# pminervini/hyperopt

Hardware: AMD Instinct MI355X
Metric: EI candidates scored/sec (x components) (higher is better)
Workload: dtype f64 (log-sum-exp: fp64 accumulation, fp32 exp2 of the shifted term, its argument from an fp32 block-local quadratic (mode 3); quantized: fp64 erf); 1 GPU; config 4: 100-D uniform space, 1e4-trial history, 1e7 candidates/suggest (lpdf roofline stress); parallelism=single

## Files before the change

### hyperopt_amd/csrc/tpe_engine.hip

```cpp
#include <hip/hip_runtime.h>

#include <algorithm>
#include <cmath>
#include <cstdlib>
#include <cstdio>
#include <cstring>
#include <string>
#include <vector>

#include "tpe_anneal.hpp"
#include "tpe_group_plan.hpp"
#include "tpe_internal.hpp"
#include "tpe_level_plan.hpp"
#include "tpe_pareto_plan.hpp"
#include "tpe_hv_plan.hpp"
#include "tpe_switches.hpp"

using namespace tpe;
static_assert(sizeof(AnnealTrace) == sizeof(tpe_anneal_trace), "layout");

struct tpe_engine {
  int32_t device = 0;
  hipStream_t stream = nullptr;
  static constexpr int kAux = 4;
// ... 697 lines not shown
  return TPE_OK;
}

StepShape step_shape(const tpe_plan *p, int64_t n_sug, int64_t n_cand, int64_t cand_begin,
                     int64_t n_total, int32_t last_nb, const FitVariant &f) {
  StepShape s;
  s.n_sug = n_sug;
  s.n_cand = n_cand;
  s.cand_begin = cand_begin;
  s.n_total = n_total;
  s.below = below_class(last_nb >= 0 ? (int64_t)last_nb + 1 : p->kcap);
  s.fit = f;
  s.prune_mode = p->prune_mode;
  s.lattice_on = p->lattice_on;
  s.screen_run = step_screen_run(switches());
  s.table_lean = switches().table_lean;
  return s;
}

int run_level(tpe_engine *h, tpe_plan *p, int level, const StepShape &s, hipStream_t st) {
  const LevelPlan lp = plan_level(*p, switches(), s, level);
  const int64_t n_sug = s.n_sug;
  const int32_t n_level = lp.n_level, n_lat = lp.n_lat;
  const int32_t *lvl = p->d_level_hps + p->level_off[level];
  if (lp.empty) {
    if (n_level > 0) CKH(launch_merge(lvl, n_level, (int32_t)n_sug, p->P, 0, nullptr, p->d_results, st));
    return TPE_OK;
  }
  ScoreArgs la = base_args(p, n_sug);
  la.level_hps = lvl;
// ... 117 lines not shown
      case Draw::Plain:
        CKH(launch_draw(a, c.table_draw, st));
        break;
      default: {
        hipError_t e;
        if (c.draw == Draw::Sorted) {
          e = launch_draw_sorted(a, c.small_table, c.fast, p->d_cpos, st);
        } else {
          rc = table_build(h, p, st);
          if (rc) { join_lk(); return rc; }
          p->tab_pstride = a.pstride;
          e = launch_draw_sorted(a, c.small_table, c.fast, p->d_cpos, st, 1);
          if (e == hipSuccess) e = launch_table_pilot(a, st);
          if (c.draw == Draw::SortedScreened) {
            if (e == hipSuccess)
              e = launch_draw_zone(a, p->d_draw_zone, c.screen_tiles, kScreenMargin, c.screen_guide,
                                   st);
            if (e == hipSuccess)
              e = launch_draw_screened(a, p->d_cpos, p->d_draw_zone, p->d_screen_stats,
                                       c.screen_guide >= 0, c.screen_run, st);
          } else if (e == hipSuccess) {
            e = launch_draw_pruned(a, c.small_table, c.fast, p->d_cpos, st);
          }
        }
        if (e != hipSuccess) { join_lk(); return fail(h, TPE_E_HIP, hipGetErrorString(e)); }
        p->dump_cn = cn;
        p->dump_sstride = a.cand_sstride;
        p->dump_level = level;
        p->dump_nsug = n_sug;
      }
    }
    a.tab_pref = c.tab_pref;
    if (c.bucket) CKH(launch_bucket(a, n_lat, p->d_cpos, st));
    a.cand_pos = c.cand_pos ? p->d_cpos : nullptr;
    if (!joined) {
// ... 2659 lines not shown
```

### hyperopt_amd/csrc/tpe_internal.hpp

```cpp
#pragma once
#include <hip/hip_runtime.h>
#include <stdint.h>

#include "../../include/tpe_engine.h"

namespace tpe {

constexpr double kEPS = 1e-12;
constexpr int kFitThreads = 1024;
constexpr int kScoreThreads = 256;
constexpr int kMaxLeaves = 160;

enum { KIND_LSE_G = 0, KIND_LSE_L = 1, KIND_ERF_G = 2, KIND_ERF_L = 3, KIND_CAT = 4,
       KIND_LAT = 5, KIND_LSE_G1 = 6, KIND_LSE_L1 = 7, KIND_LSE_GW = 8, KIND_LSE_LW = 9,
       KIND_LSE_GW1 = 10, KIND_LSE_LW1 = 11 };
constexpr int64_t kWaveRowSplitMax = (int64_t)1 << 18;

__host__ __device__ constexpr bool kind_lse(int k) {
  return k == KIND_LSE_G || k == KIND_LSE_L || k == KIND_LSE_G1 || k == KIND_LSE_L1 ||
         k == KIND_LSE_GW || k == KIND_LSE_LW || k == KIND_LSE_GW1 || k == KIND_LSE_LW1;
}
__host__ __device__ constexpr bool kind_logn(int k) {
  return k == KIND_LSE_L || k == KIND_LSE_L1 || k == KIND_LSE_LW || k == KIND_LSE_LW1 ||
         k == KIND_ERF_L;
// ... 309 lines not shown
constexpr int kZoneEdges = 2 * kZoneMax - 2;
constexpr double kScreenMargin = 1.6e-5;
constexpr int kGuideBitsMax = 10;
struct __attribute__((aligned(16))) DrawZone {
  int32_t nz;
  int32_t gbits;
  double gap_lo[kZoneMax - 1];
  double gap_hi[kZoneMax - 1];
  double thr[kFuseTab][kZoneEdges];
  uint64_t thrI[kFuseTab][kZoneEdges];
  uint64_t pickB[kFuseTab];
  uint16_t guide[1 << kGuideBitsMax];
  double tcdf[kFuseTab], tbase[kFuseTab], tmass[kFuseTab];
  unsigned char tmode[kFuseTab];
};
hipError_t launch_draw_zone(const ScoreArgs &a, DrawZone *zones, int32_t tiles, double margin,
                            int32_t guide_bits, hipStream_t st);
constexpr int kScreenRunMax = 16;
hipError_t launch_draw_screened(const ScoreArgs &a, int32_t *pos_out, const DrawZone *zones,
                                unsigned long long *stats, bool integer, int32_t run,
                                hipStream_t st);
bool is_screen_draw_kernel_fn(const void *f);
bool is_screen_run_kernel_fn(const void *f);
hipError_t launch_table_pilot(const ScoreArgs &a, hipStream_t st);
static_assert(kSortedBlock == TPE_SHARD_ALIGN, "shard alignment is the sorted-draw block");
hipError_t launch_sort_ext(const ScoreArgs &a, const double *src, int32_t *pos_out,
                           hipStream_t st);
hipError_t launch_bucket(const ScoreArgs &a, int32_t slot_begin, int32_t *pos_out, hipStream_t st);
hipError_t launch_publish(const void *src, void *dst, size_t bytes, uint64_t *flag, uint64_t seq,
                          hipStream_t st);
hipError_t launch_merge(const int32_t *level_hps, int32_t n_slots,
                        int32_t n_suggest, int32_t n_hp, int32_t world,
                        const Partial *gathered, Partial *results,
                        hipStream_t st, Partial *out2 = nullptr);
hipError_t launch_sample(const tpe_hp *hp_dev, const double *mw,
// ... 335 lines not shown
```

### hyperopt_amd/csrc/tpe_level_plan.hpp

```cpp
#pragma once
#include <algorithm>
#include <cstdint>
#include <utility>
#include <vector>

#include "tpe_internal.hpp"
#include "tpe_switches.hpp"

namespace tpe {

constexpr int64_t kSortedDrawMin = (int64_t)1 << 22;
constexpr int64_t kSmallSortMin = 2048;
constexpr int64_t kTileDrawMax = 4096;

inline int32_t active_bound(const std::vector<tpe_hp> &all, const std::vector<int32_t> &cond_parent,
                            const std::vector<int32_t> &cond_branch, const int32_t *hps, int b,
                            int e) {
  int32_t n = 0;
  std::vector<std::pair<int32_t, int32_t>> pb;
  for (int i = b; i < e; ++i) {
    const tpe_hp &x = all[hps[i]];
    if (x.cond_count == 0) { ++n; continue; }
    std::vector<std::pair<int32_t, int32_t>> mine;
    for (int c = 0; c < x.cond_count; ++c)
// ... 115 lines not shown
  f.mom_w = moments ? mom_width(ps, sw, n_hist) : 0;
  f.mom_h = f.mom_w == 16;
  return f;
}

struct StepShape {
  int64_t n_sug = 0, n_cand = 0, cand_begin = 0;
  int64_t n_total = 0;
  int32_t below = BELOW_LARGE;
  FitVariant fit;
  int32_t prune_mode = 3;
  bool lattice_on = true;
  bool capturing = false;
  bool publish = false;
  int32_t screen_run = 0;
  bool table_lean = true;
  bool operator==(const StepShape &o) const {
    return n_sug == o.n_sug && n_cand == o.n_cand && cand_begin == o.cand_begin &&
           n_total == o.n_total && below == o.below && fit == o.fit &&
           prune_mode == o.prune_mode && lattice_on == o.lattice_on &&
           capturing == o.capturing && publish == o.publish && screen_run == o.screen_run &&
           table_lean == o.table_lean;
  }
};
inline int32_t step_screen_run(const Switches &sw) {
  return sw.draw_screen && sw.draw_screen_int ? (int32_t)sw.draw_screen_run : 0;
}

struct ScoreGrid {
  int32_t n_groups = 0, pstride = 1;
  int32_t grp_kind[kMaxGroups] = {}, grp_slot0[kMaxGroups] = {}, grp_tiles[kMaxGroups] = {};
  int32_t grp_block0[kMaxGroups + 1] = {}, grp_slots[kMaxGroups] = {};
  int32_t blocks() const { return grp_block0[n_groups]; }
};
template <typename Kind, typename Rows>
ScoreGrid score_grid(Kind kind, int n_slots, int64_t cn, Rows rows) {
  ScoreGrid g;
  int32_t blocks = 0;
  auto weight = [](int k) {
    if (k == KIND_ERF_G || k == KIND_ERF_L) return 0;
    if (kind_lse(k)) return 1;
// ... 47 lines not shown
  SortedPruned,
  SortedScreened,
};

struct ChunkPlan {
  int64_t c0 = 0, cn = 0;
  bool accumulate = false;
  ScoreGrid grid;
  int32_t sort_log2 = 0, lse_pos = 0, lse_prune = 0, lse_f32 = 0, lookup_draw = 0;
  bool lk_fork = false;
  Draw draw = Draw::Plain;
  bool table_draw = false;
  bool small_table = false;
  bool fast = false;
  int32_t screen_tiles = 0;
  int32_t screen_guide = -1;
  int32_t screen_run = 0;
  bool bucket = false;
  bool cand_pos = false;
  int32_t tab_on = 0, tab_pref = 0;
  int classes = 7;
  bool publish = false;
};

struct LevelPlan {
  bool empty = false;
  int32_t n_level = 0;
  int32_t n_lat = 0;
  int32_t lat_rows = 0;
  bool compact = false;
// ... 102 lines not shown
      c.draw = Draw::Fused;
    } else if (sorted) {
      c.fast = true;
      for (int i = 0; i < n_level && c.fast; ++i) {
        const tpe_hp &x = ps.hps[hl[i]];
        const bool lookup = i < n_lat || L.kinds[i] == KIND_CAT;
        c.fast = lookup ? c.lookup_draw != 0
                        : (x.family != TPE_CAT && (x.flags & TPE_HAS_LOW) && (x.flags & TPE_HAS_HIGH));
      }
      const bool prune = c.tab_on == 1 && c.tab_pref && (cls & 1) && sw.draw_prune &&
                         c.sort_log2 == kSortLog2Large && c.cn > kSortedBlock;
      const bool screen = prune && c.fast && small_table && sw.draw_screen &&
                          c.cn * n_sug * n_level >= sw.draw_screen_min;
      c.draw = screen ? Draw::SortedScreened : prune ? Draw::SortedPruned : Draw::Sorted;
      c.screen_tiles = (int32_t)sw.draw_screen_tiles;
      c.screen_guide = sw.draw_screen_int ? (int32_t)sw.draw_screen_guide_bits : -1;
      c.screen_run = screen && c.screen_guide >= 0 ? s.screen_run : 0;
      if (prune) c.tab_pref = 2;
    } else {
      c.draw = Draw::Plain;
    }
    c.bucket = (lp.erf_level || small_sort) && !sorted;
    c.cand_pos = lp.erf_level || sorted || small_sort;
    lp.chunks.push_back(c);
  }
  return lp;
}

}
```

### hyperopt_amd/csrc/tpe_screen.hip

```cpp
#include <float.h>
#include <math.h>

#include "tpe_draw.hpp"
#include "tpe_internal.hpp"
#include "tpe_philox_row.hpp"

namespace tpe {

constexpr double kScreenQMin = 0x1p-24;
constexpr int kScreenThreads = 512;
constexpr int kZoneThreads = 256;
constexpr int kZoneCand = kHotIv + 2;
constexpr int kScreenList = 640;

__device__ __forceinline__ bool zone_crossed(double u1, double b, double m, int md, double z,
                                             double tail, bool up) {
  double pu, pp, q1;
  {
#pragma clang fp contract(off)
    const double um = u1 * m;
    pu = b - um;
    pp = b + um;
    q1 = 1.0 - pp;
  }
// ... 4 lines not shown
    above = pu < t_lo;
    below = pu > t_hi;
  } else if (md == 2 || z < 0.0) {
    above = pp > t_hi;
    below = pp < t_lo;
  } else {
    above = pp >= 0.5 && q1 < t_lo;
    below = pp < 0.5 || q1 > t_hi;
  }
  const bool ok_lo = md == 1 || pp >= kScreenQMin;
  const bool deep_hi = md == 1 ? pu < kScreenQMin : md == 0 && pp >= 0.5 && q1 < kScreenQMin;
  return deep_hi || (ok_lo && (up ? above : !below));
}

__global__ __launch_bounds__(kZoneThreads) void k_draw_zone(ScoreArgs A, DrawZone *zones,
                                                            int32_t tiles, double margin,
                                                            int32_t gbits) {
  __shared__ DrawTableT<kFuseTab> T;
  __shared__ double tmin[kPilotWaves], tmax[kPilotWaves];
  __shared__ double zlo[kZoneCand], zhi[kZoneCand];
  __shared__ uint64_t pb[kFuseTab];
  __shared__ int nz_s, bad_s;
  const int s = blockIdx.y;
  const int slot = row_slot(A, s, 0, A.n_slots, blockIdx.x);
  if (slot < 0) return;
  const int hp = A.level_hps[slot];
  const tpe_hp H = A.hps[hp];
  if (!A.force_active && !A.compact &&
      !hp_active(H, A.results + (int64_t)s * A.n_hp, A.cond_parent, A.cond_branch))
    return;
  const int kind = slot_kind(A, slot);
  if ((kind == KIND_CAT || kind == KIND_LAT) && lookup_inline(A, A.info[2 * hp].K)) return;
  DrawZone *Z = zones + ((int64_t)s * A.n_hp + hp);
  const int t = threadIdx.x, lane = t & 63, wv = t >> 6;
// ... 10 lines not shown
  }
  if (!scr) {
    if (t == 0) Z->nz = 0;
    return;
  }
  const double *pc = A.cand + (int64_t)s * A.cand_sstride + (int64_t)slot * A.n_cand;
  for (int w = wv; w < kPilotWaves; w += kZoneThreads / 64) {
    const double a = pc[w * 128 + lane], b = pc[w * 128 + 64 + lane];
    double mn = fmin(a, b), mx = fmax(a, b);
#pragma unroll
    for (int o = 32; o > 0; o >>= 1) {
      mn = fmin(mn, __shfl_xor(mn, o, 64));
      mx = fmax(mx, __shfl_xor(mx, o, 64));
    }
    if (lane == 0) { tmin[w] = mn; tmax[w] = mx; }
  }
  __syncthreads();
  if (t == 0) {
    const double pm = H.prior_mu, y_lo = hot->y_lo, y_hi = hot->y_hi;
    int nz = 0;
    zlo[nz] = -INFINITY; zhi[nz] = tmax[0]; ++nz;
    zlo[nz] = tmin[kPilotWaves - 1]; zhi[nz] = INFINITY; ++nz;
    for (int j = 0; j < nh; ++j) {
      const double l = hot->lo[j], h = hot->hi[j];
      const double a = l <= y_lo ? -INFINITY : (l + pm) - 8.0 * DBL_EPSILON * (fabs(l) + fabs(pm));
      const double b = h >= y_hi ? INFINITY : (h + pm) + 8.0 * DBL_EPSILON * (fabs(h) + fabs(pm));
      int tf = 0, tl = kPilotWaves - 1;
      while (tf < kPilotWaves && !(tmax[tf] >= a)) ++tf;
      while (tl >= 0 && !(tmin[tl] <= b)) --tl;
      double za = a, zb = b;
      if (a != -INFINITY) {
        const int w = tf - tiles;
        za = w < 0 ? -INFINITY : w < kPilotWaves ? fmin(a, tmin[w]) : a;
      }
      if (b != INFINITY) {
        const int w = tl + tiles;
        zb = w >= kPilotWaves ? INFINITY : w >= 0 ? fmax(b, tmax[w]) : b;
      }
      zlo[nz] = za; zhi[nz] = zb; ++nz;
    }
    for (int i = 1; i < nz; ++i)
      for (int j = i; j > 0 && zlo[j] < zlo[j - 1]; --j) {
        const double a = zlo[j], b = zhi[j];
        zlo[j] = zlo[j - 1]; zhi[j] = zhi[j - 1];
        zlo[j - 1] = a; zhi[j - 1] = b;
      }
    int m = 0;
    for (int i = 1; i < nz; ++i) {
      if (zlo[i] <= zhi[m]) zhi[m] = fmax(zhi[m], zhi[i]);
      else { ++m; zlo[m] = zlo[i]; zhi[m] = zhi[i]; }
    }
    nz = m + 1;
// ... 103 lines not shown
    double run = 0.0;
    for (int e = 0; e < E; ++e) {
      run = fmax(run, Z->thr[k][e]);
      Z->thr[k][e] = run;
    }
    if (gbits >= 0) {
      uint64_t runI = 0;
      for (int e = 0; e < E; ++e) {
        runI = max(runI, Z->thrI[k][e]);
        Z->thrI[k][e] = runI;
      }
    }
  }
}

hipError_t launch_draw_zone(const ScoreArgs &a, DrawZone *zones, int32_t tiles, double margin,
                            int32_t guide_bits, hipStream_t st) {
  const int64_t sbk = (int64_t)1 << a.sort_log2;
  if (a.n_slots <= 0 || a.n_suggest <= 0 || a.n_cand <= sbk) return hipSuccess;
  if (sbk != kSortedBlock || sbk != kPilotWaves * 128 || !zones || !a.tab_hot || !a.tab_hdr ||
      tiles < 0 || guide_bits > kGuideBitsMax)
    return hipErrorInvalidValue;
  k_draw_zone<<<dim3((unsigned)a.slot_rows, a.n_suggest), kZoneThreads, 0, st>>>(
      a, zones, tiles, margin, guide_bits < 0 ? -1 : guide_bits);
  return hipGetLastError();
}

template <int NT>
struct ScreenLds {
  DrawTableT<kFuseTab> T;
  union {
    double thr[kFuseTab * kZoneEdges];
    uint64_t thrI[kFuseTab * kZoneEdges];
  };
  uint32_t cnt[NT / 64 * kSortBuckets / 2];
  double red[2][NT / 64];
  unsigned char hotb[kSortBuckets], liveb[kSortBuckets];
  unsigned long long keep;
  int fail;
  int gapc[NT / 64][kZoneMax - 1];
  int ncl[NT / 64];
  double cx[NT / 64][kScreenList];
  uint32_t ci[NT / 64][kScreenList];
  uint64_t pickB[kFuseTab];
  uint16_t guide[1 << kGuideBitsMax];
};
template <int CAP, int NT>
union ScreenUnion {
  PruneDrawLds<CAP, NT> P;
  ScreenLds<NT> S;
};
static_assert(sizeof(ScreenUnion<kFuseTab, kScreenThreads>) ==
                  sizeof(PruneDrawLds<kFuseTab, kScreenThreads>),
              "the screen's layout lies inside the pruning draw's");

__device__ __forceinline__ int screen_bucket(double key, double lo, double scale) {
  int b = kSortBuckets - 1;
  if (fabs(key) < INFINITY) b = min(kSortBuckets - 1, max(0, (int)((key - lo) * scale)));
  return b;
}

template <int NT>
__device__ __forceinline__ bool screen_compose(const ScoreArgs &A, int s, int hp, int64_t base,
                                               int64_t off, int n, int nz, int ncl, double lo,
                                               double hi, double mu, const TabHot *hot,
                                               double y_lo, double y_hi, int nh,
                                               const DrawZone *__restrict__ Z,
                                               int32_t *__restrict__ pos_out, ScreenLds<NT> &L,
                                               int t) {
  constexpr int NW = NT / 64;
  const int lane = t & 63, wv = t >> 6;
  double *cx = L.cx[wv];
  uint32_t *ci = L.ci[wv];
  uint32_t *mine = L.cnt + wv * (kSortBuckets / 2);
  double *out = const_cast<double *>(A.cand) + off;
  const double scale = hi > lo ? (double)kSortBuckets / (hi - lo) : 0.0;
#pragma unroll 1
  for (int j0 = 0; j0 < ncl; j0 += 64) {
    const int j = j0 + lane;
    if (j < ncl) {
      const double x = cx[j];
      const int b = screen_bucket(x, lo, scale);
      ci[j] = (ci[j] & 0xffffu) | ((uint32_t)b << 16);
      __hip_atomic_fetch_add(&mine[b >> 1], 1u << ((b & 1) * 16), __ATOMIC_RELAXED,
                             __HIP_MEMORY_SCOPE_WORKGROUP);
      const double y = x - mu;
      const double yc = fmin(fmax(y, y_lo), y_hi);
      bool hit = y != y;
      for (int q = 0; q < nh; ++q) hit |= yc >= hot->lo[q] && yc <= hot->hi[q];
      if (hit) L.hotb[b] = 1;
    }
  }
  if (lane < nz - 1) {
    const int c = L.gapc[wv][lane];
    if (c > 0) {
      const int b = screen_bucket(Z->gap_lo[lane], lo, scale);
      __hip_atomic_fetch_add(&mine[b >> 1], (uint32_t)c << ((b & 1) * 16), __ATOMIC_RELAXED,
                             __HIP_MEMORY_SCOPE_WORKGROUP);
    }
  }
  __syncthreads();
  bucket_bases_scan<NW>(L.cnt);
  int bb = 0, be = 0;
  if (t < kSortBuckets) {
    bb = (int)((L.cnt[t >> 1] >> ((t & 1) * 16)) & 0xffffu);
// ... 249 lines not shown
      (uint32_t)__builtin_amdgcn_readfirstlane((int)(uint32_t)b)));
}

struct RunSlot {
  int hp, K, nz, gsh, nh;
  uint32_t k0, k1;
  double low, high, high_prev, mu, y_lo, y_hi;
  double gap_first, gap_last;
  const double *bmu, *bsg;
  const TabHot *hot;
  uint64_t m0lane;
};

template <int NT>
__device__ __forceinline__ void run_slot_lds(const DrawZone *__restrict__ Z, int K, int nz, int G,
                                             ScreenLds<NT> &L, int t) {
  const int E = 2 * (nz - 1);
  if (t < K) {
    L.T.cdf[t] = Z->tcdf[t];
    L.T.base[t] = Z->tbase[t];
    L.T.mass[t] = Z->tmass[t];
    L.T.mode[t] = Z->tmode[t];
  }
  for (int idx = t; idx < K * kZoneEdges; idx += NT)
    L.thrI[idx] = u53_word_threshold(idx % kZoneEdges < E ? (&Z->thrI[0][0])[idx] : 1ull << 53);
  for (int idx = t; idx < (1 << G); idx += NT) L.guide[idx] = Z->guide[idx];
  if (t < kFuseTab) L.pickB[t] = u53_word_threshold(Z->pickB[t]);
}

template <int CAP, int NT>
__device__ __forceinline__ bool screened_block_run(const ScoreArgs &A, const RunSlot &R, int slot,
                                                   int s, int64_t base,
                                                   int32_t *__restrict__ pos_out,
                                                   const DrawZone *__restrict__ Z,
                                                   ScreenLds<NT> &L, int t, int &nexact) {
  constexpr int NW = NT / 64;
  const int lane = t & 63, wv = t >> 6;
  const int nz = R.nz, E = 2 * (nz - 1), gsh = R.gsh;
  const int n = (int)min<int64_t>((int64_t)1 << A.sort_log2, A.n_cand - base);
  const int64_t off = (int64_t)s * A.cand_sstride + (int64_t)slot * A.n_cand + base;
  const int per = ((n + NW * 64 - 1) / (NW * 64)) * 64;
  const int r0 = __builtin_amdgcn_readfirstlane(wv * per);
  const int r1 = __builtin_amdgcn_readfirstlane(min(n, wv * per + per));
  const uint64_t below = lane ? (~0ull >> (64 - lane)) : 0ull;
  double *cx = L.cx[wv];
// ... 47 lines not shown
    ncl += __popcll(bal);
#pragma unroll
    for (int g = 0; g < kZoneMax - 1; ++g) {
      if (g >= nz - 1) continue;
      gc[g] += __popcll(__builtin_amdgcn_ballot_w64(c == 2 * g + 1) & vm);
    }
  }
  const bool over = ncl > kScreenList;
  if (over) ncl = 0;
  if (lane == 0) {
    L.ncl[wv] = ncl;
#pragma unroll
    for (int g = 0; g < kZoneMax - 1; ++g) L.gapc[wv][g] = gc[g];
    if (over) L.fail = 1;
  }
  double lo = INFINITY, hi = -INFINITY;
#pragma unroll 1
  for (int j0 = 0; j0 < ncl; j0 += 64) {
    const int j = j0 + lane;
    const bool v = j < ncl;
    const double u1 = u53_word_value(v ? (uint64_t)__double_as_longlong(cx[j]) : 1ull << 58);
    const int k = v ? (int)(ci[j] >> 16) : 0;
    const double x = draw_bounded_invert<CAP>(L.T, k, u1, R.bmu, R.bsg, R.low, R.high, R.high_prev,
                                              false, false, 0.0);
    if (v) {
      cx[j] = x;
      if (fabs(x) < INFINITY) { lo = fmin(lo, x); hi = fmax(hi, x); }
    }
  }
#pragma unroll
  for (int o = 32; o > 0; o >>= 1) {
    lo = fmin(lo, __shfl_xor(lo, o, 64));
    hi = fmax(hi, __shfl_xor(hi, o, 64));
  }
  if (lane == 0) { L.red[0][wv] = lo; L.red[1][wv] = hi; }
  uint32_t *mine = L.cnt + wv * (kSortBuckets / 2);
  for (int b = lane; b < kSortBuckets / 2; b += 64) mine[b] = 0u;
  __syncthreads();
  lo = INFINITY; hi = -INFINITY;
  nexact = 0;
#pragma unroll
  for (int w = 0; w < NW; ++w) {
    lo = fmin(lo, L.red[0][w]);
    hi = fmax(hi, L.red[1][w]);
    nexact += L.ncl[w];
  }
  if (L.fail || !(lo <= R.gap_first) || !(hi >= R.gap_last)) return false;
  return screen_compose<NT>(A, s, R.hp, base, off, n, nz, ncl, lo, hi, R.mu, R.hot, R.y_lo, R.y_hi,
                            R.nh, Z, pos_out, L, t);
}

template <int CAP, bool FAST>
__device__ __forceinline__ void draw_sorted_screen_run_body(const ScoreArgs &A,
                                                            int32_t *__restrict__ pos_out,
                                                            const DrawZone *__restrict__ zones,
                                                            unsigned long long *stats, int run) {
  static_assert(CAP == kFuseTab && FAST, "the small-table inline draw only");
  __shared__ __attribute__((aligned(16))) ScreenUnion<CAP, kScreenThreads> U;
  const int s = blockIdx.z;
  const int slot = row_slot(A, s, 0, A.n_slots, blockIdx.y);
  if (slot < 0) return;
  const int hp = A.level_hps[slot];
  if (!A.force_active && !A.compact &&
      !hp_active(A.hps[hp], A.results + (int64_t)s * A.n_hp, A.cond_parent, A.cond_branch))
    return;
  const int kind = slot_kind(A, slot);
  if ((kind == KIND_CAT || kind == KIND_LAT) && lookup_inline(A, A.info[2 * hp].K)) return;
// ... 26 lines not shown
    R.bmu = A.mmu + sb * A.kcap;
    R.bsg = A.msig + sb * A.kcap;
    R.hot = A.tab_hot + ((int64_t)s * A.n_hp + hp);
    R.y_lo = run_uniform(R.hot->y_lo);
    R.y_hi = run_uniform(R.hot->y_hi);
    while (R.nh < kHotIv && R.hot->lo[R.nh] <= R.hot->hi[R.nh]) ++R.nh;
    R.nh = run_uniform(R.nh);
    R.gap_first = run_uniform(Z->gap_lo[0]);
    R.gap_last = run_uniform(Z->gap_hi[nz - 2]);
    R.m0lane = philox_row_lane_term(threadIdx.x & 63);
  }
  unsigned long long screened = 0ull;
  static_assert(kScreenRunMax <= 31, "a run's sort blocks: one mask");
  uint32_t todo = scr ? 0u : (1u << (j1 - j0)) - 1u;
  if (scr) {
    run_slot_lds(Z, R.K, nz, 31 - R.gsh, U.S, (int)threadIdx.x);
#pragma unroll 1
    for (int j = j0; j < j1; ++j) {
      int t = threadIdx.x;
      asm volatile("" : "+v"(t));
      if (j > j0) __syncthreads();
      if (t < kSortBuckets) U.S.hotb[t] = 0;
      if (t == 0) { U.S.keep = 0ull; U.S.fail = 0; }
      __syncthreads();
      int nexact = 0;
      if (screened_block_run<CAP, kScreenThreads>(A, R, slot, s, (int64_t)(j + 1) << A.sort_log2,
                                                  pos_out, Z, U.S, t, nexact))
        screened += (1ull << 40) | (unsigned long long)nexact;
      else
        todo |= 1u << (j - j0);
    }
  }
  const int fallen = scr ? __popc(todo) : 0;
#pragma unroll 1
  for (int j = j0; todo != 0u; ++j, todo >>= 1) {
    if (__builtin_expect_with_probability(!(todo & 1u), 1, 0.9999999)) continue;
    __syncthreads();
    int fslot = slot, fs = s;
    typedef PruneDrawLds<CAP, kScreenThreads> __attribute__((address_space(3))) *PruneLds;
    PruneLds lds = (PruneLds)&U.P;
    asm volatile("" : "+s"(fslot), "+s"(fs), "+v"(lds));
    sorted_block_prune_body<CAP, kScreenThreads, FAST>(A, fslot, fs, (int64_t)(j + 1) << A.sort_log2,
                                                       bucket, lg, tabk, pos_out,
                                                       *(PruneDrawLds<CAP, kScreenThreads> *)lds);
  }
  if (threadIdx.x == 0) {
    if (screened) atomicAdd(stats, screened);
    if (fallen) atomicAdd(stats + 1, (unsigned long long)fallen);
  }
}
template <int CAP, bool FAST>
__global__ __launch_bounds__(kScreenThreads) __attribute__((amdgpu_waves_per_eu(4)))
void k_draw_sorted_screen_run(ScoreArgs A, int32_t *__restrict__ pos_out,
                              const DrawZone *__restrict__ zones, unsigned long long *stats,
                              int32_t run) {
  draw_sorted_screen_run_body<CAP, FAST>(A, pos_out, zones, stats, run);
}

bool is_screen_run_kernel_fn(const void *f) {
  return f == reinterpret_cast<const void *>(&k_draw_sorted_screen_run<kFuseTab, true>);
}
bool is_screen_draw_kernel_fn(const void *f) {
  return f == reinterpret_cast<const void *>(&k_draw_sorted_screen<kFuseTab, true>) ||
         f == reinterpret_cast<const void *>(&k_draw_sorted_screen_int<kFuseTab, true>) ||
         is_screen_run_kernel_fn(f);
}

hipError_t launch_draw_screened(const ScoreArgs &a, int32_t *pos_out, const DrawZone *zones,
                                unsigned long long *stats, bool integer, int32_t run,
                                hipStream_t st) {
  const int64_t sbk = (int64_t)1 << a.sort_log2;
  if (a.n_slots <= 0 || a.n_suggest <= 0 || a.n_cand <= sbk) return hipSuccess;
  if (sbk != kSortedBlock || !a.tab_wmax || !a.tab_hot || !a.tab_hdr || !zones || !stats ||
      run < 0 || run > kScreenRunMax)
    return hipErrorInvalidValue;
  const int64_t nsb = (a.n_cand + sbk - 1) / sbk - 1;
  if (integer && run >= 1) {
    const dim3 gr((unsigned)((nsb + run - 1) / run), (unsigned)a.slot_rows, a.n_suggest);
    k_draw_sorted_screen_run<kFuseTab, true><<<gr, kScreenThreads, 0, st>>>(a, pos_out, zones, stats,
                                                                            run);
    return hipGetLastError();
  }
  const dim3 g((unsigned)nsb, (unsigned)a.slot_rows, a.n_suggest);
  if (integer)
    k_draw_sorted_screen_int<kFuseTab, true><<<g, kScreenThreads, 0, st>>>(a, pos_out, zones, stats);
  else
    k_draw_sorted_screen<kFuseTab, true><<<g, kScreenThreads, 0, st>>>(a, pos_out, zones, stats);
  return hipGetLastError();
}

}
```

### hyperopt_amd/csrc/tpe_switches.hpp

```cpp
#pragma once
#include <cmath>
#include <cstdint>
#include <cstdlib>

#include "tpe_internal.hpp"

namespace tpe {

struct Switches {
  bool lookup_draw;
  bool lookup_fork;
  bool publish;
  bool tile_draw;
  bool publish_fuse;
  bool moment;
  bool table;
  bool draw_prune;
  bool draw_screen;
  bool draw_screen_int;
  bool table_prefilter;
  bool table_scalar;
  bool table_lean;
  bool small_sort;
  bool side_streams;
  bool graph;
  int64_t table_tie_log2;
  int64_t draw_screen_tiles;
  int64_t draw_screen_min;
  int64_t draw_screen_guide_bits;
  int64_t draw_screen_run;
  int64_t chunk_mb;
  int64_t lse_shift_min;

  double table_tie() const { return std::ldexp(1.0, (int)table_tie_log2); }
  int64_t chunk_budget() const { return chunk_mb << 17; }
};

constexpr int64_t kDrawScreenMin = (int64_t)1 << 26;
constexpr int64_t kDrawScreenRun = 4;

enum class SwitchRule {
  OffIfZero,
  OffIfNonEmptyZero,
  OnIfNonZero,
  OnIfSet,
  ValueIfSet,
  ValueIfNonEmpty,
};

struct SwitchDef {
  const char *name;
  SwitchRule rule;
  int64_t dflt;
  bool Switches::*flag;
  int64_t Switches::*value;
  int64_t lo, hi;
};

constexpr int64_t kTabTieLog2 = -16;
static_assert(kTabTie == 0x1p-16, "kTabTie is 2^kTabTieLog2");
// ... 10 lines not shown
      {"TPE_PUBLISH_FUSE", R::OffIfZero, 1, &S::publish_fuse, nullptr, 0, 0},
      {"TPE_MOMENT", R::OffIfZero, 1, &S::moment, nullptr, 0, 0},
      {"TPE_TABLE", R::OffIfZero, 1, &S::table, nullptr, 0, 0},
      {"TPE_DRAW_PRUNE", R::OffIfNonEmptyZero, 1, &S::draw_prune, nullptr, 0, 0},
      {"TPE_DRAW_SCREEN", R::OffIfNonEmptyZero, 1, &S::draw_screen, nullptr, 0, 0},
      {"TPE_DRAW_SCREEN_INT", R::OffIfNonEmptyZero, 1, &S::draw_screen_int, nullptr, 0, 0},
      {"TPE_TABLE_PREFILTER", R::OffIfNonEmptyZero, 1, &S::table_prefilter, nullptr, 0, 0},
      {"TPE_TABLE_SCALAR", R::OffIfNonEmptyZero, 1, &S::table_scalar, nullptr, 0, 0},
      {"TPE_TABLE_LEAN", R::OffIfNonEmptyZero, 1, &S::table_lean, nullptr, 0, 0},
      {"TPE_SMALL_SORT", R::OnIfNonZero, 0, &S::small_sort, nullptr, 0, 0},
      {"TPE_SIDE_STREAMS", R::OnIfSet, 0, &S::side_streams, nullptr, 0, 0},
      {"TPE_GRAPH", R::OnIfSet, 0, &S::graph, nullptr, 0, 0},
      {"TPE_TABLE_TIE_LOG2", R::ValueIfSet, kTabTieLog2, nullptr, &S::table_tie_log2, -1074, 4096},
      {"TPE_DRAW_SCREEN_TILES", R::ValueIfNonEmpty, 2, nullptr, &S::draw_screen_tiles, 0,
       kPilotWaves},
      {"TPE_DRAW_SCREEN_MIN", R::ValueIfNonEmpty, kDrawScreenMin, nullptr, &S::draw_screen_min, lo,
       hi},
      {"TPE_DRAW_SCREEN_GUIDE_BITS", R::ValueIfNonEmpty, 9, nullptr, &S::draw_screen_guide_bits, 0,
       kGuideBitsMax},
      {"TPE_DRAW_SCREEN_RUN", R::ValueIfNonEmpty, kDrawScreenRun, nullptr, &S::draw_screen_run, 0,
       kScreenRunMax},
      {"TPE_CHUNK_MB", R::ValueIfSet, 8192, nullptr, &S::chunk_mb, lo, hi},
      {"TPE_SHIFT_MIN_K", R::ValueIfSet, 512, nullptr, &S::lse_shift_min, lo, hi},
  };
  *n = (int)(sizeof(defs) / sizeof(defs[0]));
  return defs;
}

template <typename Get>
Switches read_switches(Get get) {
  Switches s{};
  int n = 0;
  const SwitchDef *defs = switch_table(&n);
  for (int i = 0; i < n; ++i) {
    const SwitchDef &d = defs[i];
    const char *e = get(d.name);
    switch (d.rule) {
      case SwitchRule::OffIfZero: s.*d.flag = !(e && std::atoi(e) == 0); break;
      case SwitchRule::OffIfNonEmptyZero: s.*d.flag = !(e && *e && std::atoi(e) == 0); break;
      case SwitchRule::OnIfNonZero: s.*d.flag = e && std::atoi(e) != 0; break;
      case SwitchRule::OnIfSet: s.*d.flag = e != nullptr; break;
      case SwitchRule::ValueIfSet:
      case SwitchRule::ValueIfNonEmpty: {
        const bool set = e && (d.rule == SwitchRule::ValueIfSet || *e);
        const int64_t v = set ? (int64_t)std::atoll(e) : d.dflt;
        s.*d.value = v < d.lo ? d.lo : v > d.hi ? d.hi : v;
        break;
      }
    }
  }
  return s;
}

inline const Switches &switches() {
  static const Switches s = read_switches([](const char *name) { return std::getenv(name); });
  return s;
// ... 4 lines not shown
```

Measured before the change: 1274000 billion pairs/s.

## Tighten screened-draw zones with half-wave bounds and tail quantiles; add pooled work

The zone-building kernel now tracks min/max per half-wave, giving twice as many finer pilot intervals, and widens hot intervals by a configurable number of halves instead of whole tiles. It replaces the extreme tails with a rank-selected quantile (default 24 of 128), so the tail zones are narrower. The goal is fewer candidates falling into the exact (slow) zones during screened drawing. The screened run kernel also caches the hot intervals in LDS, and gains an optional pooled mode that spreads work across waves; that mode is off by default. Narrower zones may raise the fallback rate when pilot samples are unrepresentative.

```diff
diff --git a/hyperopt_amd/csrc/tpe_engine.hip b/hyperopt_amd/csrc/tpe_engine.hip
--- a/hyperopt_amd/csrc/tpe_engine.hip
+++ b/hyperopt_amd/csrc/tpe_engine.hip
@@ -735,6 +735,9 @@
   s.prune_mode = p->prune_mode;
   s.lattice_on = p->lattice_on;
   s.screen_run = step_screen_run(switches());
+  s.screen_halves = step_screen_halves(switches());
+  s.screen_tail = (int32_t)switches().draw_screen_tail;
+  s.screen_pool = switches().draw_screen_pool;
   s.table_lean = switches().table_lean;
   return s;
 }
@@ -882,11 +885,11 @@
           if (e == hipSuccess) e = launch_table_pilot(a, st);
           if (c.draw == Draw::SortedScreened) {
             if (e == hipSuccess)
-              e = launch_draw_zone(a, p->d_draw_zone, c.screen_tiles, kScreenMargin, c.screen_guide,
-                                   st);
+              e = launch_draw_zone(a, p->d_draw_zone, c.screen_tiles, c.screen_halves, c.screen_tail,
+                                   kScreenMargin, c.screen_guide, st);
             if (e == hipSuccess)
               e = launch_draw_screened(a, p->d_cpos, p->d_draw_zone, p->d_screen_stats,
-                                       c.screen_guide >= 0, c.screen_run, st);
+                                       c.screen_guide >= 0, c.screen_run, c.screen_pool, st);
           } else if (e == hipSuccess) {
             e = launch_draw_pruned(a, c.small_table, c.fast, p->d_cpos, st);
           }
diff --git a/hyperopt_amd/csrc/tpe_internal.hpp b/hyperopt_amd/csrc/tpe_internal.hpp
--- a/hyperopt_amd/csrc/tpe_internal.hpp
+++ b/hyperopt_amd/csrc/tpe_internal.hpp
@@ -347,11 +347,11 @@
   double tcdf[kFuseTab], tbase[kFuseTab], tmass[kFuseTab];
   unsigned char tmode[kFuseTab];
 };
-hipError_t launch_draw_zone(const ScoreArgs &a, DrawZone *zones, int32_t tiles, double margin,
-                            int32_t guide_bits, hipStream_t st);
+hipError_t launch_draw_zone(const ScoreArgs &a, DrawZone *zones, int32_t tiles, int32_t halves,
+                            int32_t tail, double margin, int32_t guide_bits, hipStream_t st);
 constexpr int kScreenRunMax = 16;
 hipError_t launch_draw_screened(const ScoreArgs &a, int32_t *pos_out, const DrawZone *zones,
-                                unsigned long long *stats, bool integer, int32_t run,
+                                unsigned long long *stats, bool integer, int32_t run, bool pool,
                                 hipStream_t st);
 bool is_screen_draw_kernel_fn(const void *f);
 bool is_screen_run_kernel_fn(const void *f);
diff --git a/hyperopt_amd/csrc/tpe_level_plan.hpp b/hyperopt_amd/csrc/tpe_level_plan.hpp
--- a/hyperopt_amd/csrc/tpe_level_plan.hpp
+++ b/hyperopt_amd/csrc/tpe_level_plan.hpp
@@ -153,17 +153,24 @@
   bool capturing = false;
   bool publish = false;
   int32_t screen_run = 0;
+  int32_t screen_halves = (int32_t)kDrawScreenHalves, screen_tail = (int32_t)kDrawScreenTail;
+  bool screen_pool = false;
   bool table_lean = true;
   bool operator==(const StepShape &o) const {
     return n_sug == o.n_sug && n_cand == o.n_cand && cand_begin == o.cand_begin &&
            n_total == o.n_total && below == o.below && fit == o.fit &&
            prune_mode == o.prune_mode && lattice_on == o.lattice_on &&
            capturing == o.capturing && publish == o.publish && screen_run == o.screen_run &&
-           table_lean == o.table_lean;
+           screen_halves == o.screen_halves && screen_tail == o.screen_tail &&
+           screen_pool == o.screen_pool && table_lean == o.table_lean;
   }
 };
 inline int32_t step_screen_run(const Switches &sw) {
   return sw.draw_screen && sw.draw_screen_int ? (int32_t)sw.draw_screen_run : 0;
+}
+
+inline int32_t step_screen_halves(const Switches &sw) {
+  return sw.draw_screen_whole ? -1 : (int32_t)sw.draw_screen_halves;
 }
 
 struct ScoreGrid {
@@ -241,6 +248,9 @@
   bool small_table = false;
   bool fast = false;
   int32_t screen_tiles = 0;
+  int32_t screen_halves = 0;
+  int32_t screen_tail = 128;
+  bool screen_pool = false;
   int32_t screen_guide = -1;
   int32_t screen_run = 0;
   bool bucket = false;
@@ -373,6 +383,9 @@
                           c.cn * n_sug * n_level >= sw.draw_screen_min;
       c.draw = screen ? Draw::SortedScreened : prune ? Draw::SortedPruned : Draw::Sorted;
       c.screen_tiles = (int32_t)sw.draw_screen_tiles;
+      c.screen_halves = s.screen_halves;
+      c.screen_tail = s.screen_tail;
+      c.screen_pool = s.screen_pool;
       c.screen_guide = sw.draw_screen_int ? (int32_t)sw.draw_screen_guide_bits : -1;
       c.screen_run = screen && c.screen_guide >= 0 ? s.screen_run : 0;
       if (prune) c.tab_pref = 2;
diff --git a/hyperopt_amd/csrc/tpe_screen.hip b/hyperopt_amd/csrc/tpe_screen.hip
--- a/hyperopt_amd/csrc/tpe_screen.hip
+++ b/hyperopt_amd/csrc/tpe_screen.hip
@@ -4,6 +4,7 @@
 #include "tpe_draw.hpp"
 #include "tpe_internal.hpp"
 #include "tpe_philox_row.hpp"
+#include "tpe_screen_pool.hpp"
 
 namespace tpe {
 
@@ -42,10 +43,13 @@
 }
 
 __global__ __launch_bounds__(kZoneThreads) void k_draw_zone(ScoreArgs A, DrawZone *zones,
-                                                            int32_t tiles, double margin,
+                                                            int32_t tiles, int32_t halves,
+                                                            int32_t tail, double margin,
                                                             int32_t gbits) {
   __shared__ DrawTableT<kFuseTab> T;
   __shared__ double tmin[kPilotWaves], tmax[kPilotWaves];
+  __shared__ double hmin[2 * kPilotWaves], hmax[2 * kPilotWaves];
+  __shared__ double tail_s[2];
   __shared__ double zlo[kZoneCand], zhi[kZoneCand];
   __shared__ uint64_t pb[kFuseTab];
   __shared__ int nz_s, bad_s;
@@ -86,28 +90,60 @@
       mx = fmax(mx, __shfl_xor(mx, o, 64));
     }
     if (lane == 0) { tmin[w] = mn; tmax[w] = mx; }
+    if (halves >= 0) {
+      double an = a, ax = a, bn = b, bx = b;
+#pragma unroll
+      for (int o = 32; o > 0; o >>= 1) {
+        an = fmin(an, __shfl_xor(an, o, 64));
+        ax = fmax(ax, __shfl_xor(ax, o, 64));
+        bn = fmin(bn, __shfl_xor(bn, o, 64));
+        bx = fmax(bx, __shfl_xor(bx, o, 64));
+      }
+      if (lane == 0) { hmin[2 * w] = an; hmax[2 * w] = ax; hmin[2 * w + 1] = bn; hmax[2 * w + 1] = bx; }
+    }
+  }
+  __syncthreads();
+  static_assert(kZoneThreads >= 128, "a wave per tail");
+  if (wv < 2) {
+    const int w = wv == 0 ? 0 : kPilotWaves - 1;
+    if (lane == 0) tail_s[wv] = wv == 0 ? tmax[w] : tmin[w];
+    if (tail < 128) {
+      const double a = pc[w * 128 + lane], b = pc[w * 128 + 64 + lane];
+      int ra = 0, rb = 0;
+      for (int i = 0; i < 64; ++i) {
+        const double ua = __shfl(a, i, 64), ub = __shfl(b, i, 64);
+        ra += (ua < a || (ua == a && i < lane) ? 1 : 0) + (ub < a ? 1 : 0);
+        rb += (ua <= b ? 1 : 0) + (ub < b || (ub == b && i < lane) ? 1 : 0);
+      }
+      const int want = wv == 0 ? tail - 1 : 128 - tail;
+      if (ra == want) tail_s[wv] = a;
+      if (rb == want) tail_s[wv] = b;
+    }
   }
   __syncthreads();
   if (t == 0) {
     const double pm = H.prior_mu, y_lo = hot->y_lo, y_hi = hot->y_hi;
     int nz = 0;
-    zlo[nz] = -INFINITY; zhi[nz] = tmax[0]; ++nz;
-    zlo[nz] = tmin[kPilotWaves - 1]; zhi[nz] = INFINITY; ++nz;
+    zlo[nz] = -INFINITY; zhi[nz] = tail_s[0]; ++nz;
+    zlo[nz] = tail_s[1]; zhi[nz] = INFINITY; ++nz;
     for (int j = 0; j < nh; ++j) {
       const double l = hot->lo[j], h = hot->hi[j];
       const double a = l <= y_lo ? -INFINITY : (l + pm) - 8.0 * DBL_EPSILON * (fabs(l) + fabs(pm));
       const double b = h >= y_hi ? INFINITY : (h + pm) + 8.0 * DBL_EPSILON * (fabs(h) + fabs(pm));
-      int tf = 0, tl = kPilotWaves - 1;
-      while (tf < kPilotWaves && !(tmax[tf] >= a)) ++tf;
-      while (tl >= 0 && !(tmin[tl] <= b)) --tl;
+      const int nt = halves >= 0 ? 2 * kPilotWaves : kPilotWaves;
+      const int wide = halves >= 0 ? halves : tiles;
+      const double *vmin = halves >= 0 ? hmin : tmin, *vmax = halves >= 0 ? hmax : tmax;
+      int tf = 0, tl = nt - 1;
+      while (tf < nt && !(vmax[tf] >= a)) ++tf;
+      while (tl >= 0 && !(vmin[tl] <= b)) --tl;
       double za = a, zb = b;
       if (a != -INFINITY) {
-        const int w = tf - tiles;
-        za = w < 0 ? -INFINITY : w < kPilotWaves ? fmin(a, tmin[w]) : a;
+        const int w = tf - wide;
+        za = w < 0 ? -INFINITY : w < nt ? fmin(a, vmin[w]) : a;
       }
       if (b != INFINITY) {
-        const int w = tl + tiles;
-        zb = w >= kPilotWaves ? INFINITY : w >= 0 ? fmax(b, tmax[w]) : b;
+        const int w = tl + wide;
+        zb = w >= nt ? INFINITY : w >= 0 ? fmax(b, vmax[w]) : b;
       }
       zlo[nz] = za; zhi[nz] = zb; ++nz;
     }
@@ -241,15 +277,15 @@
   }
 }
 
-hipError_t launch_draw_zone(const ScoreArgs &a, DrawZone *zones, int32_t tiles, double margin,
-                            int32_t guide_bits, hipStream_t st) {
+hipError_t launch_draw_zone(const ScoreArgs &a, DrawZone *zones, int32_t tiles, int32_t halves,
+                            int32_t tail, double margin, int32_t guide_bits, hipStream_t st) {
   const int64_t sbk = (int64_t)1 << a.sort_log2;
   if (a.n_slots <= 0 || a.n_suggest <= 0 || a.n_cand <= sbk) return hipSuccess;
   if (sbk != kSortedBlock || sbk != kPilotWaves * 128 || !zones || !a.tab_hot || !a.tab_hdr ||
-      tiles < 0 || guide_bits > kGuideBitsMax)
+      tiles < 0 || tail < 1 || tail > 128 || guide_bits > kGuideBitsMax)
     return hipErrorInvalidValue;
   k_draw_zone<<<dim3((unsigned)a.slot_rows, a.n_suggest), kZoneThreads, 0, st>>>(
-      a, zones, tiles, margin, guide_bits < 0 ? -1 : guide_bits);
+      a, zones, tiles, halves < 0 ? -1 : halves, tail, margin, guide_bits < 0 ? -1 : guide_bits);
   return hipGetLastError();
 }
 
@@ -271,6 +307,7 @@
   uint32_t ci[NT / 64][kScreenList];
   uint64_t pickB[kFuseTab];
   uint16_t guide[1 << kGuideBitsMax];
+  double hlo[kHotIv], hhi[kHotIv];
 };
 template <int CAP, int NT>
 union ScreenUnion {
@@ -287,7 +324,7 @@
   return b;
 }
 
-template <int NT>
+template <int NT, bool POOL = false, bool HOTLDS = false>
 __device__ __forceinline__ bool screen_compose(const ScoreArgs &A, int s, int hp, int64_t base,
                                                int64_t off, int n, int nz, int ncl, double lo,
                                                double hi, double mu, const TabHot *hot,
@@ -302,20 +339,38 @@
   uint32_t *mine = L.cnt + wv * (kSortBuckets / 2);
   double *out = const_cast<double *>(A.cand) + off;
   const double scale = hi > lo ? (double)kSortBuckets / (hi - lo) : 0.0;
-#pragma unroll 1
-  for (int j0 = 0; j0 < ncl; j0 += 64) {
-    const int j = j0 + lane;
-    if (j < ncl) {
-      const double x = cx[j];
-      const int b = screen_bucket(x, lo, scale);
-      ci[j] = (ci[j] & 0xffffu) | ((uint32_t)b << 16);
-      __hip_atomic_fetch_add(&mine[b >> 1], 1u << ((b & 1) * 16), __ATOMIC_RELAXED,
-                             __HIP_MEMORY_SCOPE_WORKGROUP);
-      const double y = x - mu;
-      const double yc = fmin(fmax(y, y_lo), y_hi);
-      bool hit = y != y;
+  auto bucket_and_hot = [&](int e, uint32_t *row) {
+    const double x = (&L.cx[0][0])[e];
+    const int b = screen_bucket(x, lo, scale);
+    uint32_t *ce = &L.ci[0][0] + e;
+    *ce = (*ce & 0xffffu) | ((uint32_t)b << 16);
+    __hip_atomic_fetch_add(&row[b >> 1], 1u << ((b & 1) * 16), __ATOMIC_RELAXED,
+                           __HIP_MEMORY_SCOPE_WORKGROUP);
+    const double y = x - mu;
+    const double yc = fmin(fmax(y, y_lo), y_hi);
+    bool hit = y != y;
+    if constexpr (HOTLDS) {
+      for (int q = 0; q < nh; ++q) hit |= yc >= L.hlo[q] && yc <= L.hhi[q];
+    } else {
       for (int q = 0; q < nh; ++q) hit |= yc >= hot->lo[q] && yc <= hot->hi[q];
-      if (hit) L.hotb[b] = 1;
+    }
+    if (hit) L.hotb[b] = 1;
+  };
+  if constexpr (POOL) {
+    const int total = pool_total<NW>(L.ncl), rows = pool_rows(total);
+#pragma unroll 1
+    for (int r = wv; r < rows; r += NW) {
+      const int idx = r * 64 + lane;
+      if (idx < total) {
+        const PoolSlot o = pool_slot<NW>(L.ncl, idx);
+        bucket_and_hot(o.w * kScreenList + o.j, L.cnt + o.w * (kSortBuckets / 2));
+      }
+    }
+  } else {
+#pragma unroll 1
+    for (int j0 = 0; j0 < ncl; j0 += 64) {
+      const int j = j0 + lane;
+      if (j < ncl) bucket_and_hot(wv * kScreenList + j, mine);
     }
   }
   if (lane < nz - 1) {
@@ -595,7 +650,7 @@
 
 template <int NT>
 __device__ __forceinline__ void run_slot_lds(const DrawZone *__restrict__ Z, int K, int nz, int G,
-                                             ScreenLds<NT> &L, int t) {
+                                             const TabHot *hot, int nh, ScreenLds<NT> &L, int t) {
   const int E = 2 * (nz - 1);
   if (t < K) {
     L.T.cdf[t] = Z->tcdf[t];
@@ -607,9 +662,10 @@
     L.thrI[idx] = u53_word_threshold(idx % kZoneEdges < E ? (&Z->thrI[0][0])[idx] : 1ull << 53);
   for (int idx = t; idx < (1 << G); idx += NT) L.guide[idx] = Z->guide[idx];
   if (t < kFuseTab) L.pickB[t] = u53_word_threshold(Z->pickB[t]);
-}
-
-template <int CAP, int NT>
+  if (t < nh) { L.hlo[t] = hot->lo[t]; L.hhi[t] = hot->hi[t]; }
+}
+
+template <int CAP, int NT, bool POOL>
 __device__ __forceinline__ bool screened_block_run(const ScoreArgs &A, const RunSlot &R, int slot,
                                                    int s, int64_t base,
                                                    int32_t *__restrict__ pos_out,
@@ -687,18 +743,35 @@
     for (int g = 0; g < kZoneMax - 1; ++g) L.gapc[wv][g] = gc[g];
     if (over) L.fail = 1;
   }
+  uint32_t *mine = L.cnt + wv * (kSortBuckets / 2);
   double lo = INFINITY, hi = -INFINITY;
-#pragma unroll 1
-  for (int j0 = 0; j0 < ncl; j0 += 64) {
-    const int j = j0 + lane;
-    const bool v = j < ncl;
-    const double u1 = u53_word_value(v ? (uint64_t)__double_as_longlong(cx[j]) : 1ull << 58);
-    const int k = v ? (int)(ci[j] >> 16) : 0;
+  auto invert = [&](int e, bool v) {
+    double *xe = &L.cx[0][0] + e;
+    const double u1 = u53_word_value(v ? (uint64_t)__double_as_longlong(*xe) : 1ull << 58);
+    const int k = v ? (int)((&L.ci[0][0])[e] >> 16) : 0;
     const double x = draw_bounded_invert<CAP>(L.T, k, u1, R.bmu, R.bsg, R.low, R.high, R.high_prev,
                                               false, false, 0.0);
     if (v) {
-      cx[j] = x;
+      *xe = x;
       if (fabs(x) < INFINITY) { lo = fmin(lo, x); hi = fmax(hi, x); }
+    }
+  };
+  if constexpr (POOL) {
+    for (int b = lane; b < kSortBuckets / 2; b += 64) mine[b] = 0u;
+    __syncthreads();
+    const int total = pool_total<NW>(L.ncl), rows = pool_rows(total);
+#pragma unroll 1
+    for (int r = wv; r < rows; r += NW) {
+      const int idx = r * 64 + lane;
+      const bool v = idx < total;
+      const PoolSlot o = pool_slot<NW>(L.ncl, v ? idx : 0);
+      invert(o.w * kScreenList + o.j, v);
+    }
+  } else {
+#pragma unroll 1
+    for (int j0 = 0; j0 < ncl; j0 += 64) {
+      const int j = j0 + lane;
+      invert(wv * kScreenList + j, j < ncl);
     }
   }
 #pragma unroll
@@ -707,8 +780,8 @@
     hi = fmax(hi, __shfl_xor(hi, o, 64));
   }
   if (lane == 0) { L.red[0][wv] = lo; L.red[1][wv] = hi; }
-  uint32_t *mine = L.cnt + wv * (kSortBuckets / 2);
-  for (int b = lane; b < kSortBuckets / 2; b += 64) mine[b] = 0u;
+  if constexpr (!POOL)
+    for (int b = lane; b < kSortBuckets / 2; b += 64) mine[b] = 0u;
   __syncthreads();
   lo = INFINITY; hi = -INFINITY;
   nexact = 0;
@@ -719,11 +792,11 @@
     nexact += L.ncl[w];
   }
   if (L.fail || !(lo <= R.gap_first) || !(hi >= R.gap_last)) return false;
-  return screen_compose<NT>(A, s, R.hp, base, off, n, nz, ncl, lo, hi, R.mu, R.hot, R.y_lo, R.y_hi,
-                            R.nh, Z, pos_out, L, t);
-}
-
-template <int CAP, bool FAST>
+  return screen_compose<NT, POOL, true>(A, s, R.hp, base, off, n, nz, ncl, lo, hi, R.mu, R.hot,
+                                        R.y_lo, R.y_hi, R.nh, Z, pos_out, L, t);
+}
+
+template <int CAP, bool FAST, bool POOL>
 __device__ __forceinline__ void draw_sorted_screen_run_body(const ScoreArgs &A,
                                                             int32_t *__restrict__ pos_out,
                                                             const DrawZone *__restrict__ zones,
@@ -780,7 +853,7 @@
   static_assert(kScreenRunMax <= 31, "a run's sort blocks: one mask");
   uint32_t todo = scr ? 0u : (1u << (j1 - j0)) - 1u;
   if (scr) {
-    run_slot_lds(Z, R.K, nz, 31 - R.gsh, U.S, (int)threadIdx.x);
+    run_slot_lds(Z, R.K, nz, 31 - R.gsh, R.hot, R.nh, U.S, (int)threadIdx.x);
 #pragma unroll 1
     for (int j = j0; j < j1; ++j) {
       int t = threadIdx.x;
@@ -790,7 +863,7 @@
       if (t == 0) { U.S.keep = 0ull; U.S.fail = 0; }
       __syncthreads();
       int nexact = 0;
-      if (screened_block_run<CAP, kScreenThreads>(A, R, slot, s, (int64_t)(j + 1) << A.sort_log2,
+      if (screened_block_run<CAP, kScreenThreads, POOL>(A, R, slot, s, (int64_t)(j + 1) << A.sort_log2,
                                                   pos_out, Z, U.S, t, nexact))
         screened += (1ull << 40) | (unsigned long long)nexact;
       else
@@ -815,16 +888,17 @@
     if (fallen) atomicAdd(stats + 1, (unsigned long long)fallen);
   }
 }
-template <int CAP, bool FAST>
+template <int CAP, bool FAST, bool POOL>
 __global__ __launch_bounds__(kScreenThreads) __attribute__((amdgpu_waves_per_eu(4)))
 void k_draw_sorted_screen_run(ScoreArgs A, int32_t *__restrict__ pos_out,
                               const DrawZone *__restrict__ zones, unsigned long long *stats,
                               int32_t run) {
-  draw_sorted_screen_run_body<CAP, FAST>(A, pos_out, zones, stats, run);
+  draw_sorted_screen_run_body<CAP, FAST, POOL>(A, pos_out, zones, stats, run);
 }
 
 bool is_screen_run_kernel_fn(const void *f) {
-  return f == reinterpret_cast<const void *>(&k_draw_sorted_screen_run<kFuseTab, true>);
+  return f == reinterpret_cast<const void *>(&k_draw_sorted_screen_run<kFuseTab, true, false>) ||
+         f == reinterpret_cast<const void *>(&k_draw_sorted_screen_run<kFuseTab, true, true>);
 }
 bool is_screen_draw_kernel_fn(const void *f) {
   return f == reinterpret_cast<const void *>(&k_draw_sorted_screen<kFuseTab, true>) ||
@@ -833,7 +907,7 @@
 }
 
 hipError_t launch_draw_screened(const ScoreArgs &a, int32_t *pos_out, const DrawZone *zones,
-                                unsigned long long *stats, bool integer, int32_t run,
+                                unsigned long long *stats, bool integer, int32_t run, bool pool,
                                 hipStream_t st) {
   const int64_t sbk = (int64_t)1 << a.sort_log2;
   if (a.n_slots <= 0 || a.n_suggest <= 0 || a.n_cand <= sbk) return hipSuccess;
@@ -843,8 +917,12 @@
   const int64_t nsb = (a.n_cand + sbk - 1) / sbk - 1;
   if (integer && run >= 1) {
     const dim3 gr((unsigned)((nsb + run - 1) / run), (unsigned)a.slot_rows, a.n_suggest);
-    k_draw_sorted_screen_run<kFuseTab, true><<<gr, kScreenThreads, 0, st>>>(a, pos_out, zones, stats,
-                                                                            run);
+    if (pool)
+      k_draw_sorted_screen_run<kFuseTab, true, true><<<gr, kScreenThreads, 0, st>>>(a, pos_out, zones,
+                                                                                    stats, run);
+    else
+      k_draw_sorted_screen_run<kFuseTab, true, false><<<gr, kScreenThreads, 0, st>>>(
+          a, pos_out, zones, stats, run);
     return hipGetLastError();
   }
   const dim3 g((unsigned)nsb, (unsigned)a.slot_rows, a.n_suggest);
diff --git a/hyperopt_amd/csrc/tpe_screen_pool.hpp b/hyperopt_amd/csrc/tpe_screen_pool.hpp
--- /dev/null
+++ b/hyperopt_amd/csrc/tpe_screen_pool.hpp
@@ -0,0 +1,37 @@
+#pragma once
+#include <cstdint>
+
+#if defined(__HIPCC__) || defined(__CUDACC__)
+#define TPE_POOL_HD __host__ __device__ inline __attribute__((always_inline))
+#else
+#define TPE_POOL_HD inline
+#endif
+
+namespace tpe {
+
+struct PoolSlot { int w, j; };
+
+template <int NW>
+TPE_POOL_HD int pool_total(const int *n) {
+  int sum = 0;
+#pragma unroll
+  for (int q = 0; q < NW; ++q) sum += n[q];
+  return sum;
+}
+
+template <int NW>
+TPE_POOL_HD PoolSlot pool_slot(const int *n, int idx) {
+  int w = 0, first = 0, run = 0;
+#pragma unroll
+  for (int q = 0; q + 1 < NW; ++q) {
+    run += n[q];
+    const bool past = idx >= run;
+    w = past ? q + 1 : w;
+    first = past ? run : first;
+  }
+  return PoolSlot{w, idx - first};
+}
+
+TPE_POOL_HD int pool_rows(int total) { return (total + 63) >> 6; }
+
+}
diff --git a/hyperopt_amd/csrc/tpe_switches.hpp b/hyperopt_amd/csrc/tpe_switches.hpp
--- a/hyperopt_amd/csrc/tpe_switches.hpp
+++ b/hyperopt_amd/csrc/tpe_switches.hpp
@@ -26,6 +26,10 @@
   bool graph;
   int64_t table_tie_log2;
   int64_t draw_screen_tiles;
+  bool draw_screen_whole;
+  int64_t draw_screen_halves;
+  int64_t draw_screen_tail;
+  bool draw_screen_pool;
   int64_t draw_screen_min;
   int64_t draw_screen_guide_bits;
   int64_t draw_screen_run;
@@ -38,12 +42,15 @@
 
 constexpr int64_t kDrawScreenMin = (int64_t)1 << 26;
 constexpr int64_t kDrawScreenRun = 4;
+constexpr int64_t kDrawScreenHalves = 4;
+constexpr int64_t kDrawScreenTail = 24;
 
 enum class SwitchRule {
   OffIfZero,
   OffIfNonEmptyZero,
   OnIfNonZero,
   OnIfSet,
+  OnIfNonEmpty,
   ValueIfSet,
   ValueIfNonEmpty,
 };
@@ -84,6 +91,12 @@
       {"TPE_TABLE_TIE_LOG2", R::ValueIfSet, kTabTieLog2, nullptr, &S::table_tie_log2, -1074, 4096},
       {"TPE_DRAW_SCREEN_TILES", R::ValueIfNonEmpty, 2, nullptr, &S::draw_screen_tiles, 0,
        kPilotWaves},
+      {"TPE_DRAW_SCREEN_TILES", R::OnIfNonEmpty, 0, &S::draw_screen_whole, nullptr, 0, 0},
+      {"TPE_DRAW_SCREEN_HALVES", R::ValueIfNonEmpty, kDrawScreenHalves, nullptr,
+       &S::draw_screen_halves, 0, 2 * kPilotWaves},
+      {"TPE_DRAW_SCREEN_TAIL", R::ValueIfNonEmpty, kDrawScreenTail, nullptr, &S::draw_screen_tail, 1,
+       128},
+      {"TPE_DRAW_SCREEN_POOL", R::OnIfNonZero, 0, &S::draw_screen_pool, nullptr, 0, 0},
       {"TPE_DRAW_SCREEN_MIN", R::ValueIfNonEmpty, kDrawScreenMin, nullptr, &S::draw_screen_min, lo,
        hi},
       {"TPE_DRAW_SCREEN_GUIDE_BITS", R::ValueIfNonEmpty, 9, nullptr, &S::draw_screen_guide_bits, 0,
@@ -110,6 +123,7 @@
       case SwitchRule::OffIfNonEmptyZero: s.*d.flag = !(e && *e && std::atoi(e) == 0); break;
       case SwitchRule::OnIfNonZero: s.*d.flag = e && std::atoi(e) != 0; break;
       case SwitchRule::OnIfSet: s.*d.flag = e != nullptr; break;
+      case SwitchRule::OnIfNonEmpty: s.*d.flag = e && *e; break;
       case SwitchRule::ValueIfSet:
       case SwitchRule::ValueIfNonEmpty: {
         const bool set = e && (d.rule == SwitchRule::ValueIfSet || *e);
```

After: 1328000 billion pairs/s, median of 6. 4.2% higher.
